# dotchen/LAV

Measured on AMD Instinct MI355X. Metric: frames/s full agent fwd (32k-pt LiDAR + 3 cams), higher is better.
Workload: dtype f32 (convolution contractions on the matrix cores with f32 accumulate at the error of an fp32 dot product, DESIGN 4.3: the layers on the split-operand kernel - BEV backbone, heads, crop stems, the brake net's mid-size layers - and ERFNet's persistent runs of pairs as two power-of-two-scaled fp16 pie

## Files before the change

### include/lav_amd.h

```cpp
#ifndef LAV_AMD_H
#define LAV_AMD_H

#include <stddef.h>
#include <stdint.h>

#ifdef __cplusplus
extern "C" {
#endif

#define LAV_ABI_VERSION 40

#define LAV_OK 0
#define LAV_EINVAL (-1)
#define LAV_EHIP (-2)
#define LAV_EWORKSPACE (-3)

int lav_abi_version(void);
const char *lav_last_error(void);
int lav_device_count(void);

int lav_profile_enable(int slots);
int lav_profile_reset(void);
int lav_profile_read(const char *kernel, double *total_ms, int *launches);

typedef struct lav_grid {
// ... 200 lines not shown
                         const float *scale, const float *shift, int relu_pre, int out_c_total, int out_c_offset, float *y,
                         float *amax_out, void *stream);

size_t lav_conv1d_pair_packed_weight_floats(int channels);
int lav_conv1d_pair_pack_weights(int channels, const float *h_weight, float *h_packed);
size_t lav_conv1d_pair_chain_workspace_bytes(int batch, int h);
size_t lav_conv1d_pair_chain_lds_bytes(int channels, int w, int d_b_max);
int lav_conv1d_pair_chain(int batch, int channels, int h, int w, int npairs, const int *d_a, const int *d_b, const int *residual,
                          const int *relu_post, const float *x, const float *const *wa_packed, const float *const *bias_a,
                          const float *const *wb_packed, const float *const *bias_b, const float *const *scale,
                          const float *const *shift, float *const *out, void *workspace, size_t workspace_bytes, void *stream);
int lav_conv1d_pair_chain_f16(int batch, int channels, int h, int w, int npairs, const int *d_a, const int *d_b, const int *residual,
                              const int *relu_post, const float *x, const float *const *wa_packed, const float *const *bias_a,
                              const float *const *wb_packed, const float *const *bias_b, const float *const *scale,
                              const float *const *shift, float *const *out, void *workspace, size_t workspace_bytes, void *stream);
int lav_conv1d_pair_chain_region(int row_offset, int clean_rows);
int lav_conv1d_pair_chain_status(const void *workspace, int *h_timeouts_launches2, void *stream);
size_t lav_conv1d_pair_lds_bytes(int channels, int w, int d_b);
size_t lav_conv3x3_run_f16_workspace_bytes(int channels, int h, int w, int nlayers);
size_t lav_conv3x3_run_f16_lds_bytes(int channels, int h, int w);
size_t lav_conv3x3_run_f16_weight_bytes(int channels);
int lav_conv3x3_run_f16_amax_count(int channels, int h, int w);
long lav_conv_f16_weights_offset(const lav_conv *c);
int lav_conv3x3_run_f16(int channels, int h, int w, int nlayers, const float *x, const void *const *w_f16, const float *const *scale,
                        const float *const *shift, float *out, const float *amax_in, int amax_in_count, float *amax_out, void *workspace,
                        size_t workspace_bytes, void *stream);
int lav_conv3x3_run_f16_status(const void *workspace, int *h_timeouts_launches2, void *stream);
size_t lav_conv3x3_tile_f16_lds_bytes(int channels, int h, int w, int nlayers);
int lav_conv3x3_tile_f16_amax_count(int channels, int h, int w, int nlayers);
int lav_conv3x3_tile_f16(int channels, int h, int w, int nlayers, const float *x, const void *const *w_f16, const float *const *scale,
// ... 93 lines not shown
```

### lav_amd/_lib.py

```python
from __future__ import annotations

import ctypes as C
import os

HERE = os.path.dirname(os.path.abspath(__file__))
LIB_PATH = os.environ.get("LAV_AMD_LIB") or os.path.join(HERE, "liblav_amd.so")

ABI_VERSION = 40
MAX_CAM = 4
MAX_CAM_F64 = 8


class Grid(C.Structure):
    _fields_ = [("min_x", C.c_float), ("max_x", C.c_float), ("min_y", C.c_float), ("max_y", C.c_float),
                ("ppm", C.c_float), ("nx", C.c_int), ("ny", C.c_int)]


class PointNet(C.Structure):
    _fields_ = [("w1", C.c_void_p), ("b1", C.c_void_p), ("w2", C.c_void_p), ("b2", C.c_void_p),
                ("num_input", C.c_int), ("channels", C.c_int)]


class Camera(C.Structure):
    _fields_ = [("K", C.c_float * 9), ("l2w", C.c_float * 16), ("w2c", C.c_float * 16)]


class CameraF64(C.Structure):
    _fields_ = [("l2w", C.c_double * 16), ("w2c", C.c_double * 16), ("K", C.c_double * 9)]


class Conv(C.Structure):
    _fields_ = [(n, C.c_int) for n in (
        "batch", "in_c_total", "in_c_offset", "cin", "h", "w", "cout", "kh", "kw", "stride", "pad_h", "pad_w",
        "dil_h", "dil_w", "transposed", "out_pad", "out_c_total", "out_c_offset", "relu_pre", "relu_post", "sigmoid", "target_cus")] + [("pad_value", C.c_float), ("precision", C.c_int)]


CONV_F32, CONV_BF16X6, CONV_F16X3 = 1, 2, 3


_P, _I, _Z, _F = C.c_void_p, C.c_int, C.c_size_t, C.c_float
SIGNATURES = {
    "lav_abi_version": (_I, []),
    "lav_last_error": (C.c_char_p, []),
    "lav_device_count": (_I, []),
    "lav_profile_enable": (_I, [_I]),
    "lav_profile_reset": (_I, []),
    "lav_profile_read": (_I, [C.c_char_p, C.POINTER(C.c_double), C.POINTER(_I)]),
    "lav_pillar_workspace_bytes": (_Z, [_I, _I, C.POINTER(Grid)]),
    "lav_pillar_workspace_init": (_I, [_P, _Z, _P]),
# ... 37 lines not shown
    "lav_crop_rotate_backward": (_I, [_P, _I, _P, _I, _I, _I, _P, _P, _I, _F, _I, _F, _F, _P, _P]),
    "lav_pillar_decorate": (_I, [_P, C.POINTER(_I), _I, _I, _I, C.POINTER(Grid), _P, _P, _P, _P, _P, _P, _Z, _P]),
    "lav_scatter_max": (_I, [_P, _P, _I, _I, _I, _P, _P, _P]),
    "lav_scatter_max_backward": (_I, [_P, _P, _I, _I, _I, _P, _P]),
    "lav_conv1d_pair_packed_weight_floats": (_Z, [_I]),
    "lav_conv1d_pair_pack_weights": (_I, [_I, _P, _P]),
    "lav_upconv_pointwise_packed_floats": (_Z, [_I, _I, _I]),
    "lav_upconv_pointwise_pack": (_I, [_I, _I, _I, _P, _P]),
    "lav_upconv_pointwise_parts": (_I, [_I] * 8),
    "lav_upconv_pointwise": (_I, [_I] * 8 + [_P, _P, _P, _P, _I, _I, _I, _P, _P, _P]),
    "lav_conv1d_pair_chain_workspace_bytes": (_Z, [_I, _I]),
    "lav_conv1d_pair_chain_region": (_I, [_I, _I]),
    "lav_conv1d_pair_chain_lds_bytes": (_Z, [_I, _I, _I]),
    "lav_conv1d_pair_chain": (_I, [_I, _I, _I, _I, _I, C.POINTER(_I), C.POINTER(_I), C.POINTER(_I), C.POINTER(_I), _P] + [C.POINTER(_P)] * 7 + [_P, _Z, _P]),
    "lav_conv1d_pair_chain_f16": (_I, [_I, _I, _I, _I, _I, C.POINTER(_I), C.POINTER(_I), C.POINTER(_I), C.POINTER(_I), _P] + [C.POINTER(_P)] * 7 + [_P, _Z, _P]),
    "lav_conv1d_pair_chain_status": (_I, [_P, C.POINTER(_I), _P]),
    "lav_conv1d_pair_lds_bytes": (_Z, [_I, _I, _I]),
    "lav_conv3x3_run_f16_workspace_bytes": (_Z, [_I, _I, _I, _I]),
    "lav_conv3x3_run_f16_lds_bytes": (_Z, [_I, _I, _I]),
    "lav_conv3x3_run_f16_weight_bytes": (_Z, [_I]),
    "lav_conv3x3_run_f16_amax_count": (_I, [_I, _I, _I]),
    "lav_conv_f16_weights_offset": (C.c_long, [C.POINTER(Conv)]),
    "lav_conv3x3_run_f16": (_I, [_I, _I, _I, _I, _P, C.POINTER(_P), C.POINTER(_P), C.POINTER(_P), _P, _P, _I, _P, _P, _Z, _P]),
    "lav_conv3x3_run_f16_status": (_I, [_P, C.POINTER(_I), _P]),
    "lav_conv3x3_tile_f16_lds_bytes": (_Z, [_I, _I, _I, _I]),
    "lav_conv3x3_tile_f16_amax_count": (_I, [_I, _I, _I, _I]),
    "lav_conv3x3_tile_f16": (_I, [_I, _I, _I, _I, _P, C.POINTER(_P), C.POINTER(_P), C.POINTER(_P), _P, _P, _I, _P, _P]),
    "lav_conv1d_pair": (_I, [_I, _I, _I, _I, _I, _I, _P, _P, _P, _P, _P, _P, _P, _P, _I, _P, _P]),
    "lav_gru_seq_forward": (_I, [_P, _I, _P, _P, _P, _I, _I, _I, _P, _P, _P]),
    "lav_gru_seq_backward_workspace_bytes": (_Z, [_I, _I]),
# ... 85 lines not shown
```

### lav_amd/csrc/conv_pair.hip

```cpp
#include <algorithm>
#include <cstdlib>
#include <cstring>
#include <vector>

#include <type_traits>

#include "common.hpp"
#include "split_arith.hpp"

namespace {
using namespace lav;

struct PairArgs {
    const float *x, *wA, *bA, *wB, *bB, *scale, *shift, *res, *zero_page;
    float *y;
    unsigned long long *trace;
    int B, C, H, W, dA, dB, relu_post;
    int CP;
};

__device__ __forceinline__ void load_w(const float *__restrict__ wp, int tap, int chunk, int nchunk, int half, int co, int CP, float (&a)[8]) {
    const float4 *p = reinterpret_cast<const float4 *>(wp + ((((long)tap * nchunk + chunk) * 2 + half) * CP + co) * 8);
    const float4 lo = p[0], hi = p[1];
    a[0] = lo.x; a[1] = lo.y; a[2] = lo.z; a[3] = lo.w; a[4] = hi.x; a[5] = hi.y; a[6] = hi.z; a[7] = hi.w;
// ... 676 lines not shown
        asm volatile("s_waitcnt vmcnt(0)" ::: "memory");
        __syncthreads();
        if (tid == 0) __hip_atomic_store(a.flags + n * H + y, p + 1, __ATOMIC_RELAXED, __HIP_MEMORY_SCOPE_AGENT);
        CH_MARK(7);
        if (*(volatile int *)&s_abort) return;
    }
    if constexpr (TRACE) {
        CH_MARK(7);
        tr_acc[0] = clock64() - tr_t0;
        if (tid == 0)
            for (int i = 0; i < 8; ++i) a.trace[(long)blockIdx.x * 8 + i] = tr_acc[i];
    }
#undef CH_MARK
}

struct PairChainF16Args {
    PairChainArgs c;
    const float *tA[CHAIN_MAX], *tB[CHAIN_MAX];
    unsigned long long *rowmax;
    int rm_stride;
    int dbmax;
};

template <int KS, int R, bool TRACE = false>
__global__ __launch_bounds__(256 * KS) void k_conv1d_pair_chain_f16(PairChainF16Args fa) {
    const PairChainArgs &a = fa.c;
    long long tr_acc[8] = {0, 0, 0, 0, 0, 0, 0, 0}, tr_t = 0, tr_t0 = 0;
    if constexpr (TRACE) { tr_t0 = tr_t = clock64(); }
#define CH_MARK(i) do { if constexpr (TRACE) { const long long now_ = clock64(); tr_acc[i] += now_ - tr_t; tr_t = now_; } } while (0)
    extern __shared__ __attribute__((aligned(16))) unsigned char smem_raw[];
    const int tid = threadIdx.x, lane = tid & 63, wid8 = __builtin_amdgcn_readfirstlane(tid >> 6), l31 = lane & 31, half = lane >> 5;
    const int wid = wid8 & 3, kpart = wid8 >> 2;
    const int C = a.C, W = a.W, H = a.H, CP = a.CP;
    const int n = blockIdx.x / H, y = blockIdx.x - n * H;
    const int NPG = W >> 5, npg_sh = NPG >> 1;
    const int pg = wid & (NPG - 1), cg = wid >> npg_sh;
    const int px = pg * 32 + l31;
    const bool co_ok = cg * 32 < CP;
    const int nchunk = C >> 4, nblk = CP >> 5;
    const long rm_stride = fa.rm_stride;
    const int in_piece = nchunk * 2 * 3 * W * 16;
    const int dbmax = fa.dbmax, WM = W + 2 * dbmax, mid_piece = nchunk * 2 * WM * 16;
    float *s_red = reinterpret_cast<float *>(smem_raw);
    unsigned char *s_in = smem_raw + 16384, *s_mid = s_in + 2 * in_piece;
    __shared__ int s_abort;
    __shared__ float s_epi[4][128];
    __shared__ float s_wmax[8];
    __shared__ float s_bmax[2];
    __shared__ float s_m3;
    const int ch_lo = kpart * (nchunk / KS), ch_hi = kpart == KS - 1 ? nchunk : ch_lo + nchunk / KS;
    const int nch = ch_hi - ch_lo;
    const long plane = (long)H * W;
    const long base = (long)n * C * plane + (long)y * W + px;
    if (tid == 0) s_abort = 0;
    if (blockIdx.x == 0 && tid == 0) atomicAdd(a.sticky + 1, 1);

    u32x4 wr[R][3][2];
    auto load_w = [&](const unsigned char *wp, int t, int chunk, u32x4 (&dst)[2]) {
        const unsigned char *p = wp + ((((long)t * nchunk + chunk) * nblk + cg) * 2) * 1024 + lane * 16;
        dst[0] = *reinterpret_cast<const u32x4 *>(p);
        dst[1] = *reinterpret_cast<const u32x4 *>(p + 1024);
    };
    constexpr int NTKMAX = KS == 2 ? 2 : 3;
    float v[NTKMAX][16];
    bool okr[NTKMAX];
    auto stage_load = [&](const float *src, int dA, auto ALL_ROWS_, bool coherent) __attribute__((always_inline)) -> float {
        constexpr bool all_rows = decltype(ALL_ROWS_)::value;
        constexpr int nrow = all_rows ? 3 : 2;
        constexpr int NTK = all_rows ? (KS == 2 ? 2 : 3) : (KS == 2 ? 1 : 2);
        const int ntask = nchunk * nrow * W;
        const float *xn = src + (long)n * C * plane;
// ... 55 lines not shown
    if (co_ok) {
#pragma unroll
        for (int i = 0; i < R; ++i)
#pragma unroll
            for (int t = 0; t < 3; ++t) load_w(a.wA[0], t, ch_lo + i, wr[i][t]);
    }
    float blk_in[16], own[16];
#pragma unroll
    for (int r = 0; r < 16; ++r) { blk_in[r] = a.x0[base + (long)min(cg * 32 + (r & 3) + 8 * (r >> 2) + 4 * half, C - 1) * plane]; own[r] = 0.f; }
    {
        const int ngrp = nchunk * 2, nh = 2 * dbmax;
        for (int i = tid; i < 2 * ngrp * nh; i += 256 * KS) {
            const int j = i % nh, g = (i / nh) % ngrp, pl = i / (nh * ngrp);
            *reinterpret_cast<u32x4 *>(s_mid + pl * mid_piece + (g * WM + (j < dbmax ? j : W + j)) * 16) = u32x4{0u, 0u, 0u, 0u};
        }
    }
    __syncthreads();
    {
        m3 = 0.f;
#pragma unroll
        for (int i = 0; i < 4 * KS; ++i) m3 = fmaxf(m3, s_wmax[i]);
        stage_store(std::true_type{}, 1.f / f16_scale_of(m3));
    }

    auto mma3 = [&](f32x16 &acc, const u32x4 (&w)[2], const u32x4 (&b)[2]) {
#pragma unroll
        for (int k = 0; k < 3; ++k)
            acc = __builtin_amdgcn_mfma_f32_32x32x16_f16(__builtin_bit_cast(f16x8, w[F16X3_A[k]]), __builtin_bit_cast(f16x8, b[F16X3_B[k]]), acc, 0, 0, 0);
    };
    float m_own = 0.f;
// ... 36 lines not shown
                        const bool peer_gone = !timed_out && (spins & 63) == 0 && __hip_atomic_load(a.sticky + 2, __ATOMIC_RELAXED, __HIP_MEMORY_SCOPE_AGENT) != 0;
                        if (timed_out || peer_gone) {
                            if (lane == 0) {
                                s_abort = 1;
                                if (timed_out) { atomicAdd(a.sticky, 1); __hip_atomic_store(a.sticky + 2, 1, __ATOMIC_RELAXED, __HIP_MEMORY_SCOPE_AGENT); }
                            }
                            break;
                        }
                        __builtin_amdgcn_s_sleep(1);
                    }
                }
                if (ok && lane == 0) s_m3 = fmaxf(m_own, fmaxf(finite_abs(__uint_as_float((unsigned)wu)), finite_abs(__uint_as_float((unsigned)wd))));
            }
            __syncthreads();
            if (*(volatile int *)&s_abort) {
                float *o = a.out[a.npairs - 1] + (long)n * C * plane + (long)y * W;
                for (int i = tid; i < C * W; i += 256 * KS) o[(long)(i / W) * plane + (i % W)] = __uint_as_float(0x7fc00000u);
                return;
            }
            CH_MARK(1);
            m3 = s_m3;
            const float inv = 1.f / f16_scale_of(m3);
            (void)stage_load(a.out[p - 1], dA, std::false_type{}, true);
            stage_store(std::false_type{}, inv);
            if (co_ok && kpart == 0) {
#pragma unroll
                for (int g8 = 0; g8 < 4; ++g8) {
                    unsigned pk[2][2];
#pragma unroll
                    for (int e = 0; e < 2; ++e) split2h_pair(own[4 * g8 + 2 * e] * inv, own[4 * g8 + 2 * e + 1] * inv, pk[0][e], pk[1][e]);
                    const int grp = cg * 4 + g8;
                    if (grp * 8 < C) {
// ... 107 lines not shown
        if (co_ok && kpart == 0) {
#pragma unroll
            for (int r = 0; r < 16; ++r) {
                const int co = cg * 32 + (r & 3) + 8 * (r >> 2) + 4 * half, co_ = min(co, C - 1);
                float vv = fmaf(fmaf(acc[r], fB, s_epi[1][co_]), s_epi[2][co_], s_epi[3][co_]);
                if (a.res[p]) vv += blk_in[r];
                if (a.relu[p]) vv = vv > 0.f ? vv : 0.f;
                own[r] = co < C ? vv : 0.f;
                lm = fmaxf(lm, finite_abs(own[r]));
            }
            float *yo = a.out[p];
#pragma unroll
            for (int r = 0; r < 16; ++r) {
                const int co = cg * 32 + (r & 3) + 8 * (r >> 2) + 4 * half;
                if (co < C) {
                    if (last) yo[base + co * plane] = own[r];
                    else __hip_atomic_store(yo + base + co * plane, own[r], __ATOMIC_RELAXED, __HIP_MEMORY_SCOPE_AGENT);
                }
            }
            if (!last && a.res[p]) {
#pragma unroll
                for (int r = 0; r < 16; ++r) blk_in[r] = own[r];
            }
        }
        if (last) break;
        if (kpart == 0) {
            lm = wave_finite_absmax(lm);
            if (lane == 0) s_wmax[wid] = lm;
        }
        asm volatile("s_waitcnt vmcnt(0)" ::: "memory");
        __syncthreads();
        if (wid8 == 0) {
            m_own = fmaxf(fmaxf(s_wmax[0], s_wmax[1]), fmaxf(s_wmax[2], s_wmax[3]));
            if (lane == 0)
                __hip_atomic_store(fa.rowmax + (long)p * rm_stride + n * H + y, ((unsigned long long)(p + 1) << 32) | __float_as_uint(m_own), __ATOMIC_RELAXED,
                                   __HIP_MEMORY_SCOPE_AGENT);
        }
        CH_MARK(7);
        if (*(volatile int *)&s_abort) return;
    }
    if constexpr (TRACE) {
        CH_MARK(7);
        tr_acc[0] = clock64() - tr_t0;
        if (tid == 0)
            for (int i = 0; i < 8; ++i) a.trace[(long)blockIdx.x * 8 + i] = tr_acc[i];
    }
#undef CH_MARK
}

inline size_t pair_f32_floats(int channels) {
    const int CP = (channels + 31) / 32 * 32;
    return (size_t)3 * (channels / 16) * 2 * CP * 8;
}
inline size_t pair_split_bytes(int channels) {
// ... 180 lines not shown
}

extern "C" int lav_conv1d_pair_chain_region(int row_offset, int clean_rows) {
    LAV_REQUIRE(row_offset >= 0 && clean_rows >= -1 && (clean_rows >= 0 || row_offset == 0), "lav_conv1d_pair_chain_region: offset >= 0, clean_rows >= 0 (or -1 at offset 0: the default)");
    g_chain_row_offset = row_offset; g_chain_clean_rows = clean_rows;
    return LAV_OK;
}

extern "C" size_t lav_conv1d_pair_chain_lds_bytes(int channels, int w, int d_b_max) {
    return 16384 + (size_t)channels * w * 18 + (size_t)channels * (w + 2 * d_b_max) * 6;
}

static int pair_chain_launch(bool f16, int batch, int channels, int h, int w, int npairs, const int *d_a, const int *d_b, const int *residual,
                             const int *relu_post, const float *x, const float *const *wa_packed, const float *const *bias_a,
                             const float *const *wb_packed, const float *const *bias_b, const float *const *scale,
                             const float *const *shift, float *const *out, void *workspace, size_t workspace_bytes, void *stream) {
    LAV_REQUIRE(pair_use_split(), "lav_conv1d_pair_chain: the persistent run exists for the bf16x6 kernels only (LAV_CONV_PRECISION=f32 runs the pairs one launch each)");
    LAV_REQUIRE(batch >= 1 && h >= 1 && npairs >= 1 && npairs <= CHAIN_MAX, "lav_conv1d_pair_chain: 1..%d pairs", CHAIN_MAX);
    LAV_REQUIRE(w == 32 || w == 64 || w == 128, "lav_conv1d_pair_chain: row width %d not in {32, 64, 128}", w);
    LAV_REQUIRE(channels >= 16 && channels % 16 == 0 && (channels + 31) / 32 <= 128 / w,
                "lav_conv1d_pair_chain: %d channels do not fit a %d-pixel row tile (at most %d)", channels, w, 32 * (128 / w));
    LAV_REQUIRE(d_a && d_b && residual && relu_post && x && wa_packed && bias_a && wb_packed && bias_b && scale && shift && out, "lav_conv1d_pair_chain: null argument");
    LAV_REQUIRE(workspace && workspace_bytes >= lav_conv1d_pair_chain_workspace_bytes(batch, h), "lav_conv1d_pair_chain: workspace too small");
    static const int cus = [] {
        int dev = 0, v = 256;
        if (hipGetDevice(&dev) == hipSuccess) (void)hipDeviceGetAttribute(&v, hipDeviceAttributeMultiprocessorCount, dev);
        return v > 0 ? v : 256;
    }();
    {
        int dbm = 1;
        for (int i = 0; i < npairs; ++i) dbm = std::max(dbm, d_b[i]);
        const bool two = lav_conv1d_pair_chain_lds_bytes(channels, w, dbm) <= 76 * 1024 && !(channels >= 64 && (channels / 16) % 2 == 0);
        LAV_REQUIRE(batch * h <= cus * (two ? 2 : 1), "lav_conv1d_pair_chain: %d rows exceed the %d workgroups the chip holds at once (run the pairs one launch each)",
                    batch * h, cus * (two ? 2 : 1));
    }
    PairChainArgs a;
    int dbmax = 1;
    for (int i = 0; i < CHAIN_MAX; ++i) {
        const int j = i < npairs ? i : npairs - 1;
        LAV_REQUIRE(d_a[j] >= 1 && d_b[j] >= 1 && d_b[j] <= 16 && d_a[j] < 256, "lav_conv1d_pair_chain: bad dilation");
        LAV_REQUIRE(wa_packed[j] && bias_a[j] && wb_packed[j] && bias_b[j] && scale[j] && shift[j] && out[j], "lav_conv1d_pair_chain: null argument of pair %d", j);
        a.out[i] = out[j];
        a.wA[i] = reinterpret_cast<const unsigned char *>(wa_packed[j] + pair_f32_floats(channels));
        a.wB[i] = reinterpret_cast<const unsigned char *>(wb_packed[j] + pair_f32_floats(channels));
        a.bA[i] = bias_a[j]; a.bB[i] = bias_b[j]; a.scale[i] = scale[j]; a.shift[i] = shift[j];
        a.dA[i] = (unsigned char)d_a[j]; a.dB[i] = (unsigned char)d_b[j]; a.res[i] = residual[j] ? 1 : 0; a.relu[i] = relu_post[j] ? 1 : 0;
        dbmax = std::max(dbmax, d_b[j]);
    }
    LAV_REQUIRE(!residual[0], "lav_conv1d_pair_chain: the run starts at a block boundary (its first pair has no residual)");
    const size_t cap_rows = chain_cap_rows(workspace_bytes);
    const int row_off = g_chain_row_offset, clean_rows = g_chain_clean_rows;
    LAV_REQUIRE((size_t)row_off + (size_t)batch * h <= cap_rows && (clean_rows < 0 || (size_t)clean_rows <= cap_rows),
                "lav_conv1d_pair_chain: rows %d + %d exceed the workspace's %zu counters (lav_conv1d_pair_chain_region)", row_off, batch * h, cap_rows);
    a.x0 = x; a.sticky = static_cast<int *>(workspace); a.flags = a.sticky + 64 + row_off;
    a.B = batch; a.C = channels; a.H = h; a.W = w; a.CP = (channels + 31) / 32 * 32; a.npairs = npairs;
    const char *lim = getenv("LAV_CHAIN_SPIN_LIMIT");
// ... 15 lines not shown
    if (f16) {
        PairChainF16Args fa;
        fa.c = a;
        fa.c.trace = nullptr;
        const size_t sec = pair_f32_floats(channels) + pair_split_bytes(channels) / 4;
        for (int i = 0; i < CHAIN_MAX; ++i) {
            const int j = i < npairs ? i : npairs - 1;
            fa.c.wA[i] = reinterpret_cast<const unsigned char *>(wa_packed[j] + sec);
            fa.c.wB[i] = reinterpret_cast<const unsigned char *>(wb_packed[j] + sec);
            fa.tA[i] = wa_packed[j] + sec + pair_f16_bytes(channels) / 4;
            fa.tB[i] = wb_packed[j] + sec + pair_f16_bytes(channels) / 4;
        }
        fa.rowmax = reinterpret_cast<unsigned long long *>(static_cast<char *>(workspace) + 256 + cap_rows * sizeof(int)) + row_off;
        fa.rm_stride = (int)cap_rows;
        fa.dbmax = dbmax;
        const size_t lds16 = 16384 + (size_t)channels * w * 12 + (size_t)channels * (w + 2 * dbmax) * 4;
        constexpr size_t F16_STATIC_LDS = 2064 + 64;
#define LAV_CHAIN16_CASE(KS_, R_) if (ks2 == KS_ && ring2 == R_) { \
        static size_t cap = 0; \
        if (!cap) { \
            cap = (160 * 1024 - F16_STATIC_LDS) / 16 * 16; \
            if (hipFuncSetAttribute(reinterpret_cast<const void *>(&k_conv1d_pair_chain_f16<KS_, R_>), hipFuncAttributeMaxDynamicSharedMemorySize, (int)cap) != hipSuccess) { \
                (void)hipGetLastError(); \
                cap = 152 * 1024; \
                LAV_HIP(hipFuncSetAttribute(reinterpret_cast<const void *>(&k_conv1d_pair_chain_f16<KS_, R_>), hipFuncAttributeMaxDynamicSharedMemorySize, (int)cap)); \
            } \
        } \
         \
        hipLaunchKernelGGL((k_conv1d_pair_chain_f16<KS_, R_>), dim3(batch * h), dim3(256 * KS_), \
                           std::min(cap, std::max(lds16, lav::lds_claim(lds, F16_STATIC_LDS, batch * h > cus))), st, fa); }
        static const bool want_trace16 = getenv("LAV_PAIR_CHAIN_TRACE") != nullptr;
        if (want_trace16 && ks2 == 2 && ring2 == 2 && batch * h <= 512) {
            static long long *d_trace16 = nullptr;
            if (!d_trace16) LAV_HIP(hipMalloc(&d_trace16, (size_t)512 * 8 * sizeof(long long)));
            fa.c.trace = d_trace16;
            static bool attr_t = false;
            if (!attr_t) { LAV_HIP(hipFuncSetAttribute(reinterpret_cast<const void *>(&k_conv1d_pair_chain_f16<2, 2, true>), hipFuncAttributeMaxDynamicSharedMemorySize, 152 * 1024)); attr_t = true; }
            hipLaunchKernelGGL((k_conv1d_pair_chain_f16<2, 2, true>), dim3(batch * h), dim3(512), std::max(lds16, lav::lds_claim(lds, F16_STATIC_LDS, batch * h > cus)), st, fa);
            static int runs16 = 0;
            if (++runs16 % 10 == 0) {
                std::vector<long long> hst((size_t)batch * h * 8);
                if (hipStreamSynchronize(st) == hipSuccess && hipMemcpy(hst.data(), d_trace16, hst.size() * 8, hipMemcpyDeviceToHost) == hipSuccess) {
                    double m[8] = {0, 0, 0, 0, 0, 0, 0, 0};
                    for (int i = 0; i < batch * h; ++i) for (int k = 0; k < 8; ++k) m[k] += (double)hst[(size_t)i * 8 + k];
                    const double f = 1.0 / (batch * h) / npairs;
// ... 54 lines not shown
                                     const int *relu_post, const float *x, const float *const *wa_packed, const float *const *bias_a,
                                     const float *const *wb_packed, const float *const *bias_b, const float *const *scale,
                                     const float *const *shift, float *const *out, void *workspace, size_t workspace_bytes, void *stream) {
    return pair_chain_launch(false, batch, channels, h, w, npairs, d_a, d_b, residual, relu_post, x, wa_packed, bias_a, wb_packed, bias_b, scale, shift, out,
                             workspace, workspace_bytes, stream);
}

extern "C" int lav_conv1d_pair_chain_f16(int batch, int channels, int h, int w, int npairs, const int *d_a, const int *d_b, const int *residual,
                                         const int *relu_post, const float *x, const float *const *wa_packed, const float *const *bias_a,
                                         const float *const *wb_packed, const float *const *bias_b, const float *const *scale,
                                         const float *const *shift, float *const *out, void *workspace, size_t workspace_bytes, void *stream) {
    return pair_chain_launch(true, batch, channels, h, w, npairs, d_a, d_b, residual, relu_post, x, wa_packed, bias_a, wb_packed, bias_b, scale, shift, out,
                             workspace, workspace_bytes, stream);
}

extern "C" int lav_conv1d_pair_chain_status(const void *workspace, int *h_timeouts_launches2, void *stream) {
    LAV_REQUIRE(workspace && h_timeouts_launches2, "lav_conv1d_pair_chain_status: bad argument");
    hipStream_t st = static_cast<hipStream_t>(stream);
    LAV_HIP(hipMemcpyAsync(h_timeouts_launches2, workspace, 2 * sizeof(int), hipMemcpyDeviceToHost, st));
    LAV_HIP(hipStreamSynchronize(st));
    return LAV_OK;
}
```

### lav_amd/erfnet.py

```python
from __future__ import annotations

import os

import torch
import torch.nn as nn
import torch.nn.functional as F

from . import ops
from .ops import Conv1dPair, Conv1dPairChain, ConvLayer, GroupedDeconv, infer_precision

_USE_PAIRS = os.environ.get("LAV_ERFNET_PAIRS", "1") != "0"


def _affine(bn, sl):
    s = (bn.weight.detach().double() / torch.sqrt(bn.running_var.detach().double() + bn.eps))
    t = bn.bias.detach().double() - bn.running_mean.detach().double() * s
    return s[sl].float()[None, :, None, None].contiguous(), t[sl].float()[None, :, None, None].contiguous()


class DownsamplerBlock(nn.Module):
    def __init__(self, cin, cout):
        super().__init__()
        self.conv = nn.Conv2d(cin, cout - cin, 3, stride=2, padding=1, bias=True)
        self.pool = nn.MaxPool2d(2, stride=2)
        self.bn = nn.BatchNorm2d(cout, eps=1e-3)

# ... 55 lines not shown
        a = ConvLayer.from_module(self.conv3x1_1, relu_post=True, device=device)
        b = ConvLayer.from_module(self.conv1x3_1, self.bn1, relu_post=True, device=device)
        c = ConvLayer.from_module(self.conv3x1_2, relu_post=True, device=device)
        d = ConvLayer.from_module(self.conv1x3_2, self.bn2, relu_post=True, device=device)
        p1 = Conv1dPair(self.conv3x1_1, self.conv1x3_1, self.bn1, device=device)
        p2 = Conv1dPair(self.conv3x1_2, self.conv1x3_2, self.bn2, device=device)

        def run(x):
            if _USE_PAIRS and p1.supported(x) and p2.supported(x):
                return p2(p1(x), residual=x)
            return d(c(b(a(x))), residual=x)
        run.pairs = (p1, p2)
        return run


def _chain_blocks(stages):
    out, run = [], []

    def flush():
        if not run:
            return
        blocks = list(run)
        run.clear()
        if len(blocks) == 1 or not _USE_PAIRS:
            out.extend(blocks)
            return
        pairs = [p for b in blocks for p in b.pairs]
        chain = Conv1dPairChain(pairs, [i % 2 == 1 for i in range(len(pairs))])

        def go(x):
            if chain.supported(x):
                return chain(x)
            for b in blocks:
                x = b(x)
            return x
        go.chain = chain
        out.append(go)

    for st in stages:
        if getattr(st, "pairs", None) is not None and (not run or run[-1].pairs[0].ch == st.pairs[0].ch):
            run.append(st)
        else:
            flush()
            if getattr(st, "pairs", None) is not None:
                run.append(st)
            else:
                out.append(st)
    flush()
    return out


class UpsamplerBlock(nn.Module):
    def __init__(self, cin, cout):
        super().__init__()
        self.conv = nn.ConvTranspose2d(cin, cout, 3, stride=2, padding=1, output_padding=1, bias=True)
        self.bn = nn.BatchNorm2d(cout, eps=1e-3)

    def forward(self, x):
        return F.relu(self.bn(self.conv(x)))

    def engine(self, device):
        return ConvLayer.from_module(self.conv, self.bn, relu_post=True, device=device)

# ... 38 lines not shown
        object.__setattr__(self, "_eng", None)

    def _apply(self, fn, *a, **k):
        self._drop()
        return super()._apply(fn, *a, **k)

    def train(self, mode: bool = True):
        self._drop()
        return super().train(mode)

    def _load_from_state_dict(self, *a, **k):
        self._drop()
        return super()._load_from_state_dict(*a, **k)

    def _engine(self, device, input_affine=None, softmax=False):
        key = (device, input_affine, softmax, infer_precision())
        if self._eng is None or self._eng[0] != key:
            stages = [self.encoder.initial_block.engine(device, input_affine)]
            stages += [m.engine(device) for m in self.encoder.layers]
            stages += [m.engine(device) for m in self.decoder.layers]
            stages = _chain_blocks(stages)
            stages.append(GroupedDeconv([self.decoder.output_conv], softmax=softmax, device=device))
            object.__setattr__(self, "_eng", (key, stages))
        return self._eng[1]

    def forward(self, x, input_affine=None, softmax=False):
        if self.training:
            if input_affine is not None:
                x = x * input_affine[0] + input_affine[1]
            y = self.decoder(self.encoder(x))
            return torch.softmax(y, dim=1) if softmax else y
        if not x.is_cuda:
            raise RuntimeError("ERFNet: eval-mode forward needs a tensor in HBM - lav_amd has no CPU path "
                               "(CPU evaluation for tests and baselines: oracle/camera.py)")
        shared = os.environ.get("LAV_CHAIN_SHARED_CLEAN", "1") != "0"
        cap, off, first = ops.pair_chain_capacity(x.device), 0, True
        for stage in self._engine(x.device, input_affine, softmax):
# ... 12 lines not shown
```

### lav_amd/ops.py

```python
from __future__ import annotations

import ctypes as C
import os as _os
import threading as _threading
from typing import Optional, Sequence

import numpy as np
import torch

from . import _lib
from ._lib import Camera, Conv, Grid, PointNet, check

_workspaces: dict = {}


def _stream() -> int:
    return torch.cuda.current_stream().cuda_stream


def _ptr(t: Optional[torch.Tensor]) -> Optional[int]:
    return None if t is None else t.data_ptr()


def _f32c(t: torch.Tensor, name: str) -> torch.Tensor:
# ... 1018 lines not shown
        if ch != self.ch:
            raise RuntimeError(f"Conv1dPair: input has {ch} channels, layer expects {self.ch}")
        if residual is not None:
            residual = _f32c(residual, "residual")
            if residual.shape != x.shape:
                raise RuntimeError("residual shape mismatch")
        y = torch.empty_like(x)
        check(_lib.load().lav_conv1d_pair(B, ch, h, w, self.da, self.db, _ptr(x), _ptr(self.wa), _ptr(self.ba), _ptr(self.wb),
                                          _ptr(self.bb), _ptr(self.scale), _ptr(self.shift), _ptr(residual), int(self.relu_post),
                                          _ptr(y), _stream()), "lav_conv1d_pair")
        return y


class Conv1dPairChain:

    def __init__(self, pairs, residual):
        if len(pairs) != len(residual) or not pairs or residual[0]:
            raise RuntimeError("Conv1dPairChain: one residual flag per pair, the first pair without")
        if any(p.ch != pairs[0].ch or p.scale is None for p in pairs):
            raise RuntimeError("Conv1dPairChain: pairs of one channel count, each with its BatchNorm affine")
        self.pairs, self.residual = list(pairs), [int(bool(r)) for r in residual]
        self._bufs = {}
        self.f16 = infer_precision() == _lib.CONV_F16X3 and _os.environ.get("LAV_ERFNET_F16", "1") != "0"

    def supported(self, x: torch.Tensor) -> bool:
        lib = _lib.load()
        B, ch, h, w = x.shape
        p0 = self.pairs[0]
        lds = lib.lav_conv1d_pair_chain_lds_bytes(p0.ch, w, max(p.db for p in self.pairs))
        return (_os.environ.get("LAV_CONV_PRECISION", "bf16x6") not in ("f32", "fp32") and _os.environ.get("LAV_ERFNET_CHAIN", "1") != "0"
                and len(self.pairs) <= 16 and all(p.supported(x) for p in self.pairs)
                and B * h <= _cu_count(x.device) * (2 if (lds <= 76 * 1024 and not (ch >= 64 and (ch // 16) % 2 == 0)) else 1)
                and lds <= 152 * 1024)

    def __call__(self, x: torch.Tensor) -> torch.Tensor:
        lib = _lib.load()
        x = _f32c(x, "x")
        B, ch, h, w = x.shape
        n = len(self.pairs)
        key = (B, h, w, x.device, _stream())
        bufs = self._bufs.get(key)
        if bufs is None:
            bufs = self._bufs[key] = [torch.empty_like(x) for _ in range(n - 1)]
        out = bufs + [torch.empty_like(x)]
        ws = _workspace("pair_chain", max(lib.lav_conv1d_pair_chain_workspace_bytes(B, h), lib.lav_conv1d_pair_chain_workspace_bytes(pair_chain_capacity(x.device), 1)), x.device)
        ia = lambda vals: (C.c_int * n)(*vals)
        pa = lambda ts: (C.c_void_p * n)(*[t.data_ptr() for t in ts])
        ps = self.pairs
        check((lib.lav_conv1d_pair_chain_f16 if self.f16 else lib.lav_conv1d_pair_chain)(B, ch, h, w, n, ia([p.da for p in ps]), ia([p.db for p in ps]), ia(self.residual),
                                        ia([int(p.relu_post) for p in ps]), _ptr(x), pa([p.wa for p in ps]), pa([p.ba for p in ps]),
                                        pa([p.wb for p in ps]), pa([p.bb for p in ps]), pa([p.scale for p in ps]), pa([p.shift for p in ps]),
                                        pa(out), _ptr(ws), ws.numel(), _stream()), "lav_conv1d_pair_chain")
        return out[-1]

    def timeouts(self, x_like: torch.Tensor) -> int:
        return pair_chain_status(x_like.device)[0]


# ... 386 lines not shown
```

Before: 534.7.

## Fold ERFNet output transposed conv and softmax into the persistent f16 pair chain

Adds an epilogue to the persistent f16 ERFNet pair-chain kernel that applies the final 2x2 stride-2 ConvTranspose (up to 8 classes) and optional softmax straight from registers. The final feature map no longer has to be written and then re-read by a separate GroupedDeconv launch. The fused variant stages the output weights in LDS, uses launch bounds of 2 blocks per CU, and can only be used for 16-channel runs. This adds register pressure and per-class serial loops to the tail of the persistent kernel.

```diff
diff --git a/include/lav_amd.h b/include/lav_amd.h
--- a/include/lav_amd.h
+++ b/include/lav_amd.h
@@ -8,7 +8,7 @@
 extern "C" {
 #endif
 
-#define LAV_ABI_VERSION 40
+#define LAV_ABI_VERSION 41
 
 #define LAV_OK 0
 #define LAV_EINVAL (-1)
@@ -239,6 +239,20 @@
                               const int *relu_post, const float *x, const float *const *wa_packed, const float *const *bias_a,
                               const float *const *wb_packed, const float *const *bias_b, const float *const *scale,
                               const float *const *shift, float *const *out, void *workspace, size_t workspace_bytes, void *stream);
+typedef struct lav_pair_chain_epilogue {
+    const float *weight;
+    const float *bias;
+    float *out;
+    int classes;
+    int softmax;
+    int keep_map;
+} lav_pair_chain_epilogue;
+int lav_conv1d_pair_chain_fold_serves(int channels, int w, int classes);
+int lav_conv1d_pair_chain_fold_f16(int batch, int channels, int h, int w, int npairs, const int *d_a, const int *d_b, const int *residual,
+                                   const int *relu_post, const float *x, const float *const *wa_packed, const float *const *bias_a,
+                                   const float *const *wb_packed, const float *const *bias_b, const float *const *scale,
+                                   const float *const *shift, float *const *out, void *workspace, size_t workspace_bytes,
+                                   const lav_pair_chain_epilogue *epilogue, void *stream);
 int lav_conv1d_pair_chain_region(int row_offset, int clean_rows);
 int lav_conv1d_pair_chain_status(const void *workspace, int *h_timeouts_launches2, void *stream);
 size_t lav_conv1d_pair_lds_bytes(int channels, int w, int d_b);
diff --git a/lav_amd/_lib.py b/lav_amd/_lib.py
--- a/lav_amd/_lib.py
+++ b/lav_amd/_lib.py
@@ -6,7 +6,7 @@
 HERE = os.path.dirname(os.path.abspath(__file__))
 LIB_PATH = os.environ.get("LAV_AMD_LIB") or os.path.join(HERE, "liblav_amd.so")
 
-ABI_VERSION = 40
+ABI_VERSION = 41
 MAX_CAM = 4
 MAX_CAM_F64 = 8
 
@@ -33,6 +33,10 @@
     _fields_ = [(n, C.c_int) for n in (
         "batch", "in_c_total", "in_c_offset", "cin", "h", "w", "cout", "kh", "kw", "stride", "pad_h", "pad_w",
         "dil_h", "dil_w", "transposed", "out_pad", "out_c_total", "out_c_offset", "relu_pre", "relu_post", "sigmoid", "target_cus")] + [("pad_value", C.c_float), ("precision", C.c_int)]
+
+
+class PairChainEpilogue(C.Structure):
+    _fields_ = [("weight", C.c_void_p), ("bias", C.c_void_p), ("out", C.c_void_p), ("classes", C.c_int), ("softmax", C.c_int), ("keep_map", C.c_int)]
 
 
 CONV_F32, CONV_BF16X6, CONV_F16X3 = 1, 2, 3
@@ -100,6 +104,9 @@
     "lav_conv1d_pair_chain_lds_bytes": (_Z, [_I, _I, _I]),
     "lav_conv1d_pair_chain": (_I, [_I, _I, _I, _I, _I, C.POINTER(_I), C.POINTER(_I), C.POINTER(_I), C.POINTER(_I), _P] + [C.POINTER(_P)] * 7 + [_P, _Z, _P]),
     "lav_conv1d_pair_chain_f16": (_I, [_I, _I, _I, _I, _I, C.POINTER(_I), C.POINTER(_I), C.POINTER(_I), C.POINTER(_I), _P] + [C.POINTER(_P)] * 7 + [_P, _Z, _P]),
+    "lav_conv1d_pair_chain_fold_serves": (_I, [_I, _I, _I]),
+    "lav_conv1d_pair_chain_fold_f16": (_I, [_I, _I, _I, _I, _I, C.POINTER(_I), C.POINTER(_I), C.POINTER(_I), C.POINTER(_I), _P] + [C.POINTER(_P)] * 7
+                                       + [_P, _Z, C.POINTER(PairChainEpilogue), _P]),
     "lav_conv1d_pair_chain_status": (_I, [_P, C.POINTER(_I), _P]),
     "lav_conv1d_pair_lds_bytes": (_Z, [_I, _I, _I]),
     "lav_conv3x3_run_f16_workspace_bytes": (_Z, [_I, _I, _I, _I]),
diff --git a/lav_amd/csrc/conv_pair.hip b/lav_amd/csrc/conv_pair.hip
--- a/lav_amd/csrc/conv_pair.hip
+++ b/lav_amd/csrc/conv_pair.hip
@@ -714,17 +714,25 @@
 #undef CH_MARK
 }
 
+struct PairChainEpiArgs {
+    const float *w, *bias;
+    float *y;
+    int nc, softmax, keep_map;
+};
+
 struct PairChainF16Args {
     PairChainArgs c;
     const float *tA[CHAIN_MAX], *tB[CHAIN_MAX];
     unsigned long long *rowmax;
     int rm_stride;
     int dbmax;
+    PairChainEpiArgs epi;
 };
 
-template <int KS, int R, bool TRACE = false>
-__global__ __launch_bounds__(256 * KS) void k_conv1d_pair_chain_f16(PairChainF16Args fa) {
+template <int KS, int R, bool TRACE = false, int EPI = 0>
+__global__ __launch_bounds__(256 * KS, EPI ? 2 : 1) void k_conv1d_pair_chain_f16(PairChainF16Args fa) {
     const PairChainArgs &a = fa.c;
+    const PairChainEpiArgs &ea = fa.epi;
     long long tr_acc[8] = {0, 0, 0, 0, 0, 0, 0, 0}, tr_t = 0, tr_t0 = 0;
     if constexpr (TRACE) { tr_t0 = tr_t = clock64(); }
 #define CH_MARK(i) do { if constexpr (TRACE) { const long long now_ = clock64(); tr_acc[i] += now_ - tr_t; tr_t = now_; } } while (0)
@@ -755,6 +763,18 @@
     if (tid == 0) s_abort = 0;
     if (blockIdx.x == 0 && tid == 0) atomicAdd(a.sticky + 1, 1);
 
+    float ew[EPI == 1 ? 3 : 1];
+    if constexpr (EPI == 1) {
+        static_assert(KS == 1, "the output layer follows the 16-channel run");
+#pragma unroll
+        for (int u = 0; u < 3; ++u) {
+            const int i = tid + u * 256, c = i & 15, kx = (i >> 4) & 1, co = (i >> 5) & 7, ky = (i >> 8) & 1;
+            ew[u] = 0.f;
+            if (i < 512) { if (co < ea.nc) ew[u] = ea.w[((c * ea.nc + co) * 2 + ky) * 2 + kx]; }
+            else if (i < 520 && (i & 7) < ea.nc && ea.bias) ew[u] = ea.bias[i & 7];
+        }
+    }
+
     u32x4 wr[R][3][2];
     auto load_w = [&](const unsigned char *wp, int t, int chunk, u32x4 (&dst)[2]) {
         const unsigned char *p = wp + ((((long)t * nchunk + chunk) * nblk + cg) * 2) * 1024 + lane * 16;
@@ -840,6 +860,11 @@
             const int j = i % nh, g = (i / nh) % ngrp, pl = i / (nh * ngrp);
             *reinterpret_cast<u32x4 *>(s_mid + pl * mid_piece + (g * WM + (j < dbmax ? j : W + j)) * 16) = u32x4{0u, 0u, 0u, 0u};
         }
+    }
+    if constexpr (EPI == 1) {
+#pragma unroll
+        for (int u = 0; u < 3; ++u)
+            if (tid + u * 256 < 520) s_red[tid + u * 256] = ew[u];
     }
     __syncthreads();
     {
@@ -906,8 +931,14 @@
             }
             __syncthreads();
             if (*(volatile int *)&s_abort) {
-                float *o = a.out[a.npairs - 1] + (long)n * C * plane + (long)y * W;
-                for (int i = tid; i < C * W; i += 256 * KS) o[(long)(i / W) * plane + (i % W)] = __uint_as_float(0x7fc00000u);
+                if (EPI == 0 || ea.keep_map) {
+                    float *o = a.out[a.npairs - 1] + (long)n * C * plane + (long)y * W;
+                    for (int i = tid; i < C * W; i += 256 * KS) o[(long)(i / W) * plane + (i % W)] = __uint_as_float(0x7fc00000u);
+                }
+                if constexpr (EPI == 1) {
+                    float *o = ea.y + (long)n * ea.nc * 4 * plane + (long)y * 4 * W;
+                    for (int i = tid; i < ea.nc * 4 * W; i += 256 * KS) o[(long)(i / (4 * W)) * 4 * plane + (i % (4 * W))] = __uint_as_float(0x7fc00000u);
+                }
                 return;
             }
             CH_MARK(1);
@@ -1045,7 +1076,7 @@
             for (int r = 0; r < 16; ++r) {
                 const int co = cg * 32 + (r & 3) + 8 * (r >> 2) + 4 * half;
                 if (co < C) {
-                    if (last) yo[base + co * plane] = own[r];
+                    if (last) { if (EPI == 0 || ea.keep_map) yo[base + co * plane] = own[r]; }
                     else __hip_atomic_store(yo + base + co * plane, own[r], __ATOMIC_RELAXED, __HIP_MEMORY_SCOPE_AGENT);
                 }
             }
@@ -1069,6 +1100,61 @@
         }
         CH_MARK(7);
         if (*(volatile int *)&s_abort) return;
+    }
+    if constexpr (EPI == 1) {
+        if (co_ok && kpart == 0) {
+            float xc[16];
+#pragma unroll
+            for (int j = 0; j < 8; ++j) {
+                const float other = __shfl_xor(own[j], 32);
+                const int c = 8 * (j >> 2) + (j & 3);
+                xc[c] = half ? other : own[j];
+                xc[c + 4] = half ? own[j] : other;
+            }
+            const int nc = ea.nc;
+            const float *wl = s_red + half * 256;
+            float *ssc = reinterpret_cast<float *>(s_in) + tid;
+            const int sst = 2 * W;
+            float *yp = ea.y + (long)n * nc * 4 * plane + (long)(2 * y + half) * 2 * W + 2 * px;
+            float m0 = -INFINITY, m1 = -INFINITY;
+#pragma unroll 1
+            for (int co = 0; co < nc; ++co) {
+                float s0 = 0.f, s1 = 0.f;
+                float4 wq[2][4];
+#pragma unroll
+                for (int q = 0; q < 4; ++q) {
+                    wq[0][q] = *reinterpret_cast<const float4 *>(wl + (co * 2 + 0) * 16 + 4 * q);
+                    wq[1][q] = *reinterpret_cast<const float4 *>(wl + (co * 2 + 1) * 16 + 4 * q);
+                }
+#pragma unroll
+                for (int q = 0; q < 4; ++q) {
+                    s0 = fmaf(xc[4 * q], wq[0][q].x, s0); s1 = fmaf(xc[4 * q], wq[1][q].x, s1);
+                    s0 = fmaf(xc[4 * q + 1], wq[0][q].y, s0); s1 = fmaf(xc[4 * q + 1], wq[1][q].y, s1);
+                    s0 = fmaf(xc[4 * q + 2], wq[0][q].z, s0); s1 = fmaf(xc[4 * q + 2], wq[1][q].z, s1);
+                    s0 = fmaf(xc[4 * q + 3], wq[0][q].w, s0); s1 = fmaf(xc[4 * q + 3], wq[1][q].w, s1);
+                }
+                const float b = s_red[512 + co];
+                s0 = s0 + b; s1 = s1 + b;
+                if (ea.softmax) {
+                    ssc[co * sst] = s0; ssc[(8 + co) * sst] = s1;
+                    m0 = fmaxf(m0, s0); m1 = fmaxf(m1, s1);
+                } else {
+                    *reinterpret_cast<float2 *>(yp + (long)co * 4 * plane) = float2{s0, s1};
+                }
+            }
+            if (ea.softmax) {
+                float sum0 = 0.f, sum1 = 0.f;
+#pragma unroll 1
+                for (int co = 0; co < nc; ++co) {
+                    const float e0 = expf(ssc[co * sst] - m0), e1 = expf(ssc[(8 + co) * sst] - m1);
+                    ssc[co * sst] = e0; ssc[(8 + co) * sst] = e1;
+                    sum0 += e0; sum1 += e1;
+                }
+#pragma unroll 1
+                for (int co = 0; co < nc; ++co)
+                    *reinterpret_cast<float2 *>(yp + (long)co * 4 * plane) = float2{ssc[co * sst] / sum0, ssc[(8 + co) * sst] / sum1};
+            }
+        }
     }
     if constexpr (TRACE) {
         CH_MARK(7);
@@ -1279,7 +1365,8 @@
 static int pair_chain_launch(bool f16, int batch, int channels, int h, int w, int npairs, const int *d_a, const int *d_b, const int *residual,
                              const int *relu_post, const float *x, const float *const *wa_packed, const float *const *bias_a,
                              const float *const *wb_packed, const float *const *bias_b, const float *const *scale,
-                             const float *const *shift, float *const *out, void *workspace, size_t workspace_bytes, void *stream) {
+                             const float *const *shift, float *const *out, void *workspace, size_t workspace_bytes, void *stream,
+                             const PairChainEpiArgs *epi = nullptr) {
     LAV_REQUIRE(pair_use_split(), "lav_conv1d_pair_chain: the persistent run exists for the bf16x6 kernels only (LAV_CONV_PRECISION=f32 runs the pairs one launch each)");
     LAV_REQUIRE(batch >= 1 && h >= 1 && npairs >= 1 && npairs <= CHAIN_MAX, "lav_conv1d_pair_chain: 1..%d pairs", CHAIN_MAX);
     LAV_REQUIRE(w == 32 || w == 64 || w == 128, "lav_conv1d_pair_chain: row width %d not in {32, 64, 128}", w);
@@ -1304,7 +1391,8 @@
     for (int i = 0; i < CHAIN_MAX; ++i) {
         const int j = i < npairs ? i : npairs - 1;
         LAV_REQUIRE(d_a[j] >= 1 && d_b[j] >= 1 && d_b[j] <= 16 && d_a[j] < 256, "lav_conv1d_pair_chain: bad dilation");
-        LAV_REQUIRE(wa_packed[j] && bias_a[j] && wb_packed[j] && bias_b[j] && scale[j] && shift[j] && out[j], "lav_conv1d_pair_chain: null argument of pair %d", j);
+        LAV_REQUIRE(wa_packed[j] && bias_a[j] && wb_packed[j] && bias_b[j] && scale[j] && shift[j] && (out[j] || (epi && !epi->keep_map && j == npairs - 1)),
+                    "lav_conv1d_pair_chain: null argument of pair %d", j);
         a.out[i] = out[j];
         a.wA[i] = reinterpret_cast<const unsigned char *>(wa_packed[j] + pair_f32_floats(channels));
         a.wB[i] = reinterpret_cast<const unsigned char *>(wb_packed[j] + pair_f32_floats(channels));
@@ -1350,6 +1438,7 @@
         fa.rowmax = reinterpret_cast<unsigned long long *>(static_cast<char *>(workspace) + 256 + cap_rows * sizeof(int)) + row_off;
         fa.rm_stride = (int)cap_rows;
         fa.dbmax = dbmax;
+        fa.epi = epi ? *epi : PairChainEpiArgs{nullptr, nullptr, nullptr, 0, 0, 0};
         const size_t lds16 = 16384 + (size_t)channels * w * 12 + (size_t)channels * (w + 2 * dbmax) * 4;
         constexpr size_t F16_STATIC_LDS = 2064 + 64;
 #define LAV_CHAIN16_CASE(KS_, R_) if (ks2 == KS_ && ring2 == R_) { \
@@ -1365,6 +1454,19 @@
          \
         hipLaunchKernelGGL((k_conv1d_pair_chain_f16<KS_, R_>), dim3(batch * h), dim3(256 * KS_), \
                            std::min(cap, std::max(lds16, lav::lds_claim(lds, F16_STATIC_LDS, batch * h > cus))), st, fa); }
+        if (epi) {
+            LAV_REQUIRE(ks2 == 1 && ring2 == 1, "lav_conv1d_pair_chain_fold_f16: the output layer follows a 16-channel run");
+            static size_t cap = 0;
+            if (!cap) {
+                cap = 152 * 1024;
+                LAV_HIP(hipFuncSetAttribute(reinterpret_cast<const void *>(&k_conv1d_pair_chain_f16<1, 1, false, 1>), hipFuncAttributeMaxDynamicSharedMemorySize, (int)cap));
+            }
+            hipLaunchKernelGGL((k_conv1d_pair_chain_f16<1, 1, false, 1>), dim3(batch * h), dim3(256),
+                               std::min(cap, std::max(lds16, lav::lds_claim(lds, F16_STATIC_LDS, batch * h > cus))), st, fa);
+            timer_end(tok, st);
+            LAV_LAUNCH_CHECK();
+            return LAV_OK;
+        }
         static const bool want_trace16 = getenv("LAV_PAIR_CHAIN_TRACE") != nullptr;
         if (want_trace16 && ks2 == 2 && ring2 == 2 && batch * h <= 512) {
             static long long *d_trace16 = nullptr;
@@ -1449,6 +1551,26 @@
                              workspace, workspace_bytes, stream);
 }
 
+extern "C" int lav_conv1d_pair_chain_fold_serves(int channels, int w, int classes) {
+    return channels == 16 && (w == 32 || w == 64 || w == 128) && classes >= 1 && classes <= 8;
+}
+
+extern "C" int lav_conv1d_pair_chain_fold_f16(int batch, int channels, int h, int w, int npairs, const int *d_a, const int *d_b, const int *residual,
+                                              const int *relu_post, const float *x, const float *const *wa_packed, const float *const *bias_a,
+                                              const float *const *wb_packed, const float *const *bias_b, const float *const *scale,
+                                              const float *const *shift, float *const *out, void *workspace, size_t workspace_bytes,
+                                              const lav_pair_chain_epilogue *epilogue, void *stream) {
+    LAV_REQUIRE(epilogue && epilogue->weight && epilogue->out, "lav_conv1d_pair_chain_fold_f16: null epilogue argument");
+    LAV_REQUIRE(lav_conv1d_pair_chain_fold_serves(channels, w, epilogue->classes),
+                "lav_conv1d_pair_chain_fold_f16: the output layer folds into a 16-channel run with 1..8 classes (%d channels, %d classes)", channels, epilogue->classes);
+    LAV_REQUIRE(reinterpret_cast<uintptr_t>(epilogue->out) % 8 == 0, "lav_conv1d_pair_chain_fold_f16: out must be 8-byte aligned");
+    PairChainEpiArgs ea;
+    ea.w = epilogue->weight; ea.bias = epilogue->bias; ea.y = epilogue->out;
+    ea.nc = epilogue->classes; ea.softmax = epilogue->softmax ? 1 : 0; ea.keep_map = epilogue->keep_map ? 1 : 0;
+    return pair_chain_launch(true, batch, channels, h, w, npairs, d_a, d_b, residual, relu_post, x, wa_packed, bias_a, wb_packed, bias_b, scale, shift, out,
+                             workspace, workspace_bytes, stream, &ea);
+}
+
 extern "C" int lav_conv1d_pair_chain_status(const void *workspace, int *h_timeouts_launches2, void *stream) {
     LAV_REQUIRE(workspace && h_timeouts_launches2, "lav_conv1d_pair_chain_status: bad argument");
     hipStream_t st = static_cast<hipStream_t>(stream);
diff --git a/lav_amd/erfnet.py b/lav_amd/erfnet.py
--- a/lav_amd/erfnet.py
+++ b/lav_amd/erfnet.py
@@ -10,6 +10,19 @@
 from .ops import Conv1dPair, Conv1dPairChain, ConvLayer, GroupedDeconv, infer_precision
 
 _USE_PAIRS = os.environ.get("LAV_ERFNET_PAIRS", "1") != "0"
+
+
+FOLDS = ("out",)
+FOLD_DEFAULT = "out"
+
+
+def _folds():
+    v = os.environ.get("LAV_ERFNET_FOLD", FOLD_DEFAULT).strip()
+    names = () if v in ("0", "") else tuple(n.strip() for n in v.split(","))
+    bad = [n for n in names if n not in FOLDS]
+    if bad:
+        raise RuntimeError(f"LAV_ERFNET_FOLD: {bad} not in {FOLDS}")
+    return names
 
 
 def _affine(bn, sl):
@@ -95,10 +108,10 @@
         return run
 
 
-def _chain_blocks(stages):
+def _chain_blocks(stages, epilogue=None):
     out, run = [], []
 
-    def flush():
+    def flush(epi=None):
         if not run:
             return
         blocks = list(run)
@@ -107,14 +120,16 @@
             out.extend(blocks)
             return
         pairs = [p for b in blocks for p in b.pairs]
-        chain = Conv1dPairChain(pairs, [i % 2 == 1 for i in range(len(pairs))])
+        chain = Conv1dPairChain(pairs, [i % 2 == 1 for i in range(len(pairs))], epilogue=epi)
 
         def go(x):
             if chain.supported(x):
-                return chain(x)
+                folded = chain.folded(x)
+                x = chain(x)
+                return x if folded or epi is None else epi(x)
             for b in blocks:
                 x = b(x)
-            return x
+            return x if epi is None else epi(x)
         go.chain = chain
         out.append(go)
 
@@ -127,7 +142,10 @@
                 run.append(st)
             else:
                 out.append(st)
-    flush()
+    ends_with_run = len(run) > 1 and _USE_PAIRS
+    flush(epilogue if ends_with_run else None)
+    if epilogue is not None and not ends_with_run:
+        out.append(epilogue)
     return out
 
 
@@ -196,13 +214,17 @@
         return super()._load_from_state_dict(*a, **k)
 
     def _engine(self, device, input_affine=None, softmax=False):
-        key = (device, input_affine, softmax, infer_precision())
+        folds = _folds()
+        key = (device, input_affine, softmax, infer_precision(), folds)
         if self._eng is None or self._eng[0] != key:
             stages = [self.encoder.initial_block.engine(device, input_affine)]
             stages += [m.engine(device) for m in self.encoder.layers]
             stages += [m.engine(device) for m in self.decoder.layers]
-            stages = _chain_blocks(stages)
-            stages.append(GroupedDeconv([self.decoder.output_conv], softmax=softmax, device=device))
+            tail = GroupedDeconv([self.decoder.output_conv], softmax=softmax, device=device)
+            if "out" in folds:
+                stages = _chain_blocks(stages, epilogue=tail)
+            else:
+                stages = _chain_blocks(stages) + [tail]
             object.__setattr__(self, "_eng", (key, stages))
         return self._eng[1]
 
diff --git a/lav_amd/ops.py b/lav_amd/ops.py
--- a/lav_amd/ops.py
+++ b/lav_amd/ops.py
@@ -1056,7 +1056,7 @@
 
 class Conv1dPairChain:
 
-    def __init__(self, pairs, residual):
+    def __init__(self, pairs, residual, epilogue: Optional["GroupedDeconv"] = None):
         if len(pairs) != len(residual) or not pairs or residual[0]:
             raise RuntimeError("Conv1dPairChain: one residual flag per pair, the first pair without")
         if any(p.ch != pairs[0].ch or p.scale is None for p in pairs):
@@ -1064,6 +1064,15 @@
         self.pairs, self.residual = list(pairs), [int(bool(r)) for r in residual]
         self._bufs = {}
         self.f16 = infer_precision() == _lib.CONV_F16X3 and _os.environ.get("LAV_ERFNET_F16", "1") != "0"
+        if epilogue is not None and ((epilogue.k, epilogue.s, epilogue.pad, epilogue.opad, epilogue.groups) != (2, 2, 0, 0, 1)
+                                     or epilogue.cin_g != pairs[0].ch or epilogue.sigmoid_from not in (-1, -2)):
+            raise RuntimeError("Conv1dPairChain: the epilogue is one ConvTranspose2d(channels, classes, 2, stride 2), scores or softmax")
+        self.epilogue = epilogue
+        self.last_map = None
+
+    def folded(self, x: torch.Tensor) -> bool:
+        return (self.epilogue is not None and self.f16 and self.supported(x)
+                and bool(_lib.load().lav_conv1d_pair_chain_fold_serves(x.shape[1], x.shape[3], self.epilogue.outs[0])))
 
     def supported(self, x: torch.Tensor) -> bool:
         lib = _lib.load()
@@ -1075,7 +1084,7 @@
                 and B * h <= _cu_count(x.device) * (2 if (lds <= 76 * 1024 and not (ch >= 64 and (ch // 16) % 2 == 0)) else 1)
                 and lds <= 152 * 1024)
 
-    def __call__(self, x: torch.Tensor) -> torch.Tensor:
+    def __call__(self, x: torch.Tensor, keep_map: bool = False) -> torch.Tensor:
         lib = _lib.load()
         x = _f32c(x, "x")
         B, ch, h, w = x.shape
@@ -1084,6 +1093,20 @@
         bufs = self._bufs.get(key)
         if bufs is None:
             bufs = self._bufs[key] = [torch.empty_like(x) for _ in range(n - 1)]
+        if self.folded(x):
+            e = self.epilogue
+            ws = _workspace("pair_chain", max(lib.lav_conv1d_pair_chain_workspace_bytes(B, h), lib.lav_conv1d_pair_chain_workspace_bytes(pair_chain_capacity(x.device), 1)), x.device)
+            self.last_map = torch.empty_like(x) if keep_map else None
+            y = torch.empty((B, e.outs[0], 2 * h, 2 * w), dtype=torch.float32, device=x.device)
+            ia = lambda vals: (C.c_int * n)(*vals)
+            pa = lambda ts: (C.c_void_p * n)(*[None if t is None else t.data_ptr() for t in ts])
+            ps = self.pairs
+            epi = _lib.PairChainEpilogue(_ptr(e.w), _ptr(e.bias), _ptr(y), e.outs[0], int(e.sigmoid_from == -2), int(keep_map))
+            check(lib.lav_conv1d_pair_chain_fold_f16(B, ch, h, w, n, ia([p.da for p in ps]), ia([p.db for p in ps]), ia(self.residual),
+                                                     ia([int(p.relu_post) for p in ps]), _ptr(x), pa([p.wa for p in ps]), pa([p.ba for p in ps]),
+                                                     pa([p.wb for p in ps]), pa([p.bb for p in ps]), pa([p.scale for p in ps]), pa([p.shift for p in ps]),
+                                                     pa(bufs + [self.last_map]), _ptr(ws), ws.numel(), C.byref(epi), _stream()), "lav_conv1d_pair_chain_fold_f16")
+            return y
         out = bufs + [torch.empty_like(x)]
         ws = _workspace("pair_chain", max(lib.lav_conv1d_pair_chain_workspace_bytes(B, h), lib.lav_conv1d_pair_chain_workspace_bytes(pair_chain_capacity(x.device), 1)), x.device)
         ia = lambda vals: (C.c_int * n)(*vals)
```

Measured after the change: 541.2 (median of 6 runs). 1.01x the previous value.
